# Pablete1234/parquet-floor

Hardware: AMD Instinct MI355X
Metric: decoded GB/s + rows/s (node), lineitem-shape Snappy+dict, 1/2/4/8 GPUs (higher is better)
Workload: dtype u8; 1 GPU; lineitem SF1 x1 (6001215 rows x 1, 16 cols, 6 row groups of 1Mi rows), Snappy + dictionary, device-resident; row_groups_per_rank=6, compressed_page_bytes_rank0=217870360

## Files before the change

parquet-floor_amd/csrc/pf_flat.hip:

```cpp
#include <hip/hip_runtime.h>

#include "pf_flat.h"
#include "pf_flat_chars.h"
#include "pf_launch.h"
#include "pf_snappy_par.h"

namespace pf {

#ifdef PF_STAMPS
#include "pf_stamps.h"
PF_STAMP_TABLE(pf_pstamps, 16, pf_debug_pstamps)
#define PSTAMP(i, v) atomicAdd(&pf_pstamps[i], (unsigned long long)(v))
#else
#define PSTAMP(i, v) ((void)0)
#endif

struct FlatLds {
    uint32_t dpos[DSTR_CAP], dlen[DSTR_CAP];
    Run drun[RUN_CAP];
    Run vrun[RUN_CAP];
    uint32_t coff[FT];
    uint32_t csrc[FT];
    uint16_t cv[CV_CAP];
    uint32_t vbits[FT / 32 + 2];
    uint32_t scan_tmp[NT / 64];
    RunWalk dst, vst;
    int ndrun, nvrun, dres, vres, allp;
    uint32_t dcover, vcover, vlo;
};

#ifndef PF_DICT_LDS
#define PF_DICT_LDS 16384
#endif
constexpr uint32_t DICT_LDS = PF_DICT_LDS;
#ifndef PF_FIX_IDS
#define PF_FIX_IDS 0
#endif
struct FixedLds {
    uint64_t dict[(DICT_LDS + PF_FIX_IDS) / 8 + 2];
    Run vrun[RUN_CAP];
    uint32_t coff[FTX / 64];
    RunWalk vst;
    int nvrun, vres, allp;
    uint32_t vcover, vlo;
    uint32_t ib[2];
};

template <class Lds>
__device__ __forceinline__ int flat_present_fixed(Lds& S, const DevChunk& ck, const DevPage& pg, const Sections& s, bool dict,
                                  bool boolean, int enc, int w, const uint8_t* ids, uint64_t ids_n, int id_bw,
                                  uint64_t slot_base, uint32_t e_begin, uint32_t e_end, bool direct = false) {
    const int tid = threadIdx.x;
    const uint8_t* vend = s.val + s.val_n;
    const bool dalign = dict && (reinterpret_cast<uintptr_t>(ck.dict_data) & uintptr_t(w - 1)) == 0;
    const bool dlds = DICT_LDS > 0 && dict && dalign && (w == 4 || w == 8) && ck.dict_data != nullptr &&
                      ck.dict_n > 0 && uint64_t(ck.dict_n) * uint64_t(w) <= DICT_LDS;
    const uint32_t dbytes = dlds ? (uint32_t(ck.dict_n) * uint32_t(w) + 15u) & ~15u : 0u;
    uint8_t* const sid = reinterpret_cast<uint8_t*>(S.dict) + dbytes;
    int64_t idd = 0;
    bool ilds = false;
    if (dict && dalign && (w == 4 || w == 8) && id_bw > 0 && id_bw <= 32 && s.val_n > 0 && S.vres != 2 &&
        S.vlo <= e_begin && e_end <= S.vcover) {
        if (tid == 0) { S.ib[0] = 0xffffffffu; S.ib[1] = 0u; }
        __syncthreads();
        for (int r = tid; r < S.nvrun; r += NT) {
            const Run R = S.vrun[r];
            const uint32_t f = max(R.first, e_begin), l = min(R.first + R.count, e_end);
            if (!R.packed || f >= l) continue;
            atomicMin(&S.ib[0], uint32_t((uint64_t(R.data) + uint64_t(f - R.first) * uint64_t(id_bw)) >> 3));
            atomicMax(&S.ib[1], uint32_t((uint64_t(R.data) + uint64_t(l - R.first) * uint64_t(id_bw) + 7u) >> 3));
        }
        __syncthreads();
        const uint32_t lo = S.ib[0], hi = S.ib[1];
        if (lo < hi && hi <= ids_n) {
            const uintptr_t a0 = (reinterpret_cast<uintptr_t>(ids) + lo) & ~uintptr_t(15);
            const uintptr_t aend = reinterpret_cast<uintptr_t>(ids) + ids_n;
            const uint32_t nb = (uint32_t(reinterpret_cast<uintptr_t>(ids) + hi - a0) + 8u + 15u) & ~15u;
            if (dbytes + nb <= uint32_t(sizeof(S.dict))) {
                ilds = true;
                idd = int64_t(a0) - int64_t(reinterpret_cast<uintptr_t>(ids));
                for (uint32_t c = tid; c < nb / 16u; c += NT) {
                    const uintptr_t a = a0 + 16u * c;
                    u32x4 x;
                    if (a + 16u <= aend) {
                        x = *reinterpret_cast<const PF_GLOBAL u32x4*>(a);
                    } else {
                        uint32_t q[4] = {0, 0, 0, 0};
                        for (uint32_t b = 0; b < 16u && a + b < aend; b++)
                            q[b >> 2] |= uint32_t(*reinterpret_cast<const PF_GLOBAL uint8_t*>(a + b)) << (8 * (b & 3));
                        x = u32x4{q[0], q[1], q[2], q[3]};
                    }
                    reinterpret_cast<u32x4*>(sid)[c] = x;
                }
            }
        }
    }
    if (dlds) {
        const uint32_t dn = uint32_t(ck.dict_n);
        if (w == 8) {
            const PF_GLOBAL uint64_t* g = (const PF_GLOBAL uint64_t*)(ck.dict_data);
            for (uint32_t i0 = tid; i0 < dn; i0 += 8u * NT) {
                uint64_t v[8];
                #pragma unroll
                for (uint32_t k = 0; k < 8; k++) v[k] = i0 + k * NT < dn ? g[i0 + k * NT] : 0ull;
                #pragma unroll
                for (uint32_t k = 0; k < 8; k++) if (i0 + k * NT < dn) S.dict[i0 + k * NT] = v[k];
            }
        } else {
            const PF_GLOBAL uint32_t* g = (const PF_GLOBAL uint32_t*)(ck.dict_data);
            uint32_t* d32 = reinterpret_cast<uint32_t*>(S.dict);
            for (uint32_t i0 = tid; i0 < dn; i0 += 8u * NT) {
                uint32_t v[8];
                #pragma unroll
                for (uint32_t k = 0; k < 8; k++) v[k] = i0 + k * NT < dn ? g[i0 + k * NT] : 0u;
                #pragma unroll
                for (uint32_t k = 0; k < 8; k++) if (i0 + k * NT < dn) d32[i0 + k * NT] = v[k];
            }
        }
    }
    if (dlds || ilds) __syncthreads();
    for (uint32_t e0 = e_begin, want = 0; e0 < e_end; e0 += want) {
        want = min(uint32_t(FTX), e_end - e0);
        int bad = 0;
        if (dict) {
            if ((S.vlo > e0 || e0 + want > S.vcover) && S.vres == 2) {
                __syncthreads();
                if (tid < 64) {
                    if (tid == 0) { S.vst = RunWalk{0, 0}; S.vlo = e0; }
                    const int rr = wave_walk_runs(ids, ids_n, id_bw, e0, e_end, S.vrun, RUN_CAP, S.nvrun, S.vcover, S.vst, RunWalk{0, 0});
                    if (tid == 0) S.vres = rr;
                }
                __syncthreads();
                if (S.vres == 2 && S.vcover > e0 && e0 + want > S.vcover) want = S.vcover - e0;
            }
            if (id_bw > 32 || s.val_n == 0 || ck.dict_data == nullptr || e0 + want > S.vcover || S.vlo > e0) bad = 1;
            if (!bad && uint32_t(tid) < (want + 63) / 64) S.coff[tid] = uint32_t(run_find(S.vrun, S.nvrun, e0 + tid * 64));
            __syncthreads();
        }
        const bool wide = w == 4 || w == 8;
        if (direct) {
        } else if (!bad && wide && ((dict && dalign) || enc == 0 || enc == 5)) {
#ifndef PF_FB_DIV
#define PF_FB_DIV 2
#endif
            constexpr uint32_t FB = FEPTX / PF_FB_DIV;
            for (uint32_t kb = 0; kb < FEPTX; kb += FB) {
            uint64_t v[FB];
            uint32_t id[FB];
            #pragma unroll
            for (uint32_t k = 0; k < FB; k++) {
                const uint32_t e = e0 + (kb + k) * NT + uint32_t(tid);
                id[k] = 0;
                v[k] = 0;
                if (e >= e0 + want) continue;
                if (dict) {
                    int r = int(S.coff[(e - e0) >> 6]);
                    while (e >= S.vrun[r].first + S.vrun[r].count) r++;
                    const Run R = S.vrun[r];
                    id[k] = R.data;
                    if (R.packed) {
                        const uint64_t bit = uint64_t(R.data) + uint64_t(e - R.first) * uint64_t(id_bw);
                        if (ilds) {
                            const uint32_t rb = uint32_t(int64_t(bit) - 8 * idd);
                            const uint32_t* q = reinterpret_cast<const uint32_t*>(sid) + (rb >> 5);
                            const uint64_t x = (uint64_t(q[0]) | (uint64_t(q[1]) << 32)) >> (rb & 31u);
                            id[k] = uint32_t(x & (id_bw == 32 ? 0xffffffffull : ((1ull << id_bw) - 1ull)));
                        } else {
                            id[k] = (bit >> 3) + 12 <= ids_n ? bits_fast(ids + (bit >> 3), uint32_t(bit & 7), id_bw)
                                                             : bits_le(ids, ids_n, bit, id_bw);
                        }
                    }
                } else if (enc == 0) {
                    if ((uint64_t(e) + 1) * uint64_t(w) > s.val_n) { bad = 1; continue; }
                    const uint8_t* src = s.val + uint64_t(e) * uint64_t(w);
                    if (w == 8) v[k] = src + 12 <= vend ? gld_u64_12(src) : ld64_bytes(src);
                    else v[k] = src + 8 <= vend ? gld_u32_8(src) : ld32le(src, 0, 4);
                } else {
                    v[k] = reinterpret_cast<const uint64_t*>(pg.aux)[e];
                }
            }
            if (dict) {
                const int64_t dn = ck.dict_n;
                #pragma unroll
                for (uint32_t k = 0; k < FB; k++) {
                    const uint32_t e = e0 + (kb + k) * NT + uint32_t(tid);
                    if (e < e0 + want && int64_t(id[k]) >= dn) bad = 1;
                    id[k] = int64_t(id[k]) < dn ? id[k] : 0u;
                }
                if (dlds) {
                    #pragma unroll
                    for (uint32_t k = 0; k < FB; k++)
                        v[k] = w == 8 ? S.dict[id[k]] : reinterpret_cast<const uint32_t*>(S.dict)[id[k]];
                } else if (w == 8) {
                    const PF_GLOBAL uint64_t* g = (const PF_GLOBAL uint64_t*)ck.dict_data;
                    #pragma unroll
                    for (uint32_t k = 0; k < FB; k++) v[k] = g[id[k]];
                } else {
                    const PF_GLOBAL uint32_t* g = (const PF_GLOBAL uint32_t*)ck.dict_data;
                    #pragma unroll
                    for (uint32_t k = 0; k < FB; k++) v[k] = g[id[k]];
                }
            }
            #pragma unroll
            for (uint32_t k = 0; k < FB; k++) {
                const uint32_t e = e0 + (kb + k) * NT + uint32_t(tid);
                if (e >= e0 + want) continue;
                uint8_t* dst = ck.values + (slot_base + e) * uint64_t(w);
                if (w == 8) *reinterpret_cast<uint64_t*>(dst) = v[k];
                else *reinterpret_cast<uint32_t*>(dst) = uint32_t(v[k]);
            }
            }
        } else if (!bad) {
            #pragma unroll 2
            for (uint32_t k = 0; k < FEPTX; k++) {
                const uint32_t e = e0 + k * NT + uint32_t(tid);
                if (e >= e0 + want) break;
                uint8_t* dst = ck.values + (slot_base + e) * uint64_t(w);
                if (dict) {
                    int r = int(S.coff[(e - e0) >> 6]);
                    while (e >= S.vrun[r].first + S.vrun[r].count) r++;
                    const Run R = S.vrun[r];
                    uint32_t id = R.data;
                    if (R.packed) {
                        const uint64_t bit = uint64_t(R.data) + uint64_t(e - R.first) * uint64_t(id_bw);
                        id = (bit >> 3) + 12 <= ids_n ? bits_fast(ids + (bit >> 3), uint32_t(bit & 7), id_bw)
                                                      : bits_le(ids, ids_n, bit, id_bw);
                    }
                    if (int64_t(id) >= ck.dict_n) { bad = 1; continue; }
                    const uint8_t* src = ck.dict_data + uint64_t(id) * uint64_t(w);
                    if (w == 8 && dalign) *reinterpret_cast<uint64_t*>(dst) = *reinterpret_cast<const uint64_t*>(src);
                    else if (w == 4 && dalign) *reinterpret_cast<uint32_t*>(dst) = *reinterpret_cast<const uint32_t*>(src);
                    else copy_value(dst, src, w);
                } else if (boolean) {
                    if ((e >> 3) >= s.val_n) { bad = 1; continue; }
                    dst[0] = uint8_t((s.val[e >> 3] >> (e & 7)) & 1u);
                } else if (enc == 0) {
                    if ((uint64_t(e) + 1) * uint64_t(w) > s.val_n) { bad = 1; continue; }
                    const uint8_t* src = s.val + uint64_t(e) * uint64_t(w);
                    if (w == 8 && src + 12 <= vend) *reinterpret_cast<uint64_t*>(dst) = gld_u64_12(src);
                    else if (w == 4 && src + 8 <= vend) *reinterpret_cast<uint32_t*>(dst) = gld_u32_8(src);
                    else copy_value(dst, src, w);
                } else {
                    const uint64_t* dv = reinterpret_cast<const uint64_t*>(pg.aux);
                    if (w == 8) *reinterpret_cast<uint64_t*>(dst) = dv[e];
                    else *reinterpret_cast<uint32_t*>(dst) = uint32_t(dv[e]);
                }
            }
        }
        if (ck.max_def > 0 && ck.validity) {
            const uint64_t b0 = slot_base + e0, b1 = b0 + want;
            uint32_t* vw = reinterpret_cast<uint32_t*>(ck.validity);
            for (uint64_t wd = (b0 >> 5) + tid; wd <= ((b1 - 1) >> 5); wd += NT) {
                const uint64_t lo = max(b0, wd << 5), hi = min(b1, (wd + 1) << 5);
                const uint32_t m = uint32_t((hi - lo >= 32 ? 0xffffffffull : ((1ull << (hi - lo)) - 1ull)) << (lo & 31));
                if (lo == (wd << 5) && hi == ((wd + 1) << 5)) vw[wd] = m;
                else atomicOr(vw + wd, m);
            }
        }
        if (__syncthreads_or(bad)) return 1;
    }
    return 0;
}

__device__ __forceinline__ bool flat_fixed_block(FixedLds& S, const DevChunk* __restrict__ chunks, DevPage* pages, const int2 pbk,
                                 DevChunkResult* res) {
    if (pbk.x < 0) return true;
    const int pi = pbk.x;
    const uint32_t blk = uint32_t(pbk.y) & 0x0fffffffu;
    const uint32_t bsz = FBLK << (uint32_t(pbk.y) >> 28);
    DevPage& pg = pages[pi];
    const DevChunk& ck = chunks[pg.chunk];
    const int tid = threadIdx.x;
    const int* jfb = pg.jfb;
    const bool dval = pg.direct == DIRECT_VALUES;
    const int jf = jfb != nullptr ? *jfb : FB_WHOLE + 1;
    const int done = pg.done;
    if (done & DONE_DSTR) return true;
    if ((res[pg.chunk].status != 0) | (ck.max_rep != 0) | (ck.ptype == 6) | ((done & DONE_NULL) != 0)) return false;
    if (dval & (jf <= FB_WHOLE)) {
        const uint32_t ne = uint32_t(pg.num_values), e_begin = blk * bsz;
        if (e_begin >= ne && blk > 0) return true;
        const uint32_t e_end = min(ne, e_begin + bsz);
        if (ck.max_def > 0 && ck.validity && e_end > e_begin)
            fill_valid_ones(ck, uint64_t(pg.entry_start) + e_begin, uint64_t(pg.entry_start) + e_end);
        if (threadIdx.x == 0) {
            if (ck.needs_count == 0)
                atomicAdd(reinterpret_cast<unsigned long long*>(&res[pg.chunk].num_values), (unsigned long long)(e_end - e_begin));
            atomicOr(&pg.done, DONE_FIXED);
        }
        return true;
    }
    Sections s;
    if (!page_sections(pg, ck, s)) return false;
    const int enc = pg.encoding;
    const bool boolean = ck.ptype == 0, dict = is_dict_enc(enc);
    const int w = ck.width;
    bool take = ck.max_def == 0 || s.def_rle;
    if (enc == 0) {
    } else if (dict) take = take && !boolean;
    else if (enc == 5) take = take && (ck.ptype == 1 || ck.ptype == 2) && pg.aux != nullptr;
    else take = false;
    if (!take) return false;
    const uint32_t ne = uint32_t(pg.num_values);
    if (blk > 0 && blk * bsz >= ne) return true;
    const int id_bw = (dict && s.val_n > 0) ? int(s.val[0]) : 0;
    const uint8_t* ids = dict && s.val_n > 0 ? s.val + 1 : s.val;
    const uint64_t ids_n = dict && s.val_n > 0 ? s.val_n - 1 : 0;
    const IdRunTab* T = pg.runtab;
    uint32_t t0 = 0, t3 = 0;
    if (T != nullptr) { t0 = T->nruns; t3 = T->all_present; }
    const bool tab = (t3 == 1u) & (t0 <= uint32_t(RUN_CAP));
    if (tid == 0)
        S.allp = tab ? 1 : (ck.max_def == 0 ? 1 : all_present(s.def, s.def_n, bit_width(ck.max_def), ne, uint32_t(ck.max_def)));
    __syncthreads();
    if (!S.allp) return false;
    const uint32_t e_begin = blk * bsz;
    const uint32_t e_end = min(ne, e_begin + bsz);
#ifdef PF_STAMPS
    const unsigned long long ft0 = __builtin_amdgcn_s_memtime();
#endif
    if (dict) {
        if (tab) {
            const uint32_t nr = T->nruns, cov = T->covered;
            for (uint32_t i = tid; i < nr; i += NT) S.vrun[i] = id_run(T, i, nr, cov);
            if (tid == 0) { S.nvrun = int(nr); S.vcover = cov; S.vlo = 0; S.vres = cov >= ne ? 0 : 1; }
        } else if (tid < 64) {
            if (tid == 0) { S.nvrun = 0; S.vcover = 0; S.vres = 0; S.vlo = e_begin; S.vst = RunWalk{0, 0}; }
            if (s.val_n > 0 && id_bw <= 32) {
                const int rr = wave_walk_runs(ids, ids_n, id_bw, e_begin, e_end, S.vrun, RUN_CAP, S.nvrun, S.vcover, S.vst, RunWalk{0, 0});
                if (tid == 0) S.vres = rr;
            }
        }
        __syncthreads();
    }
    const bool direct = dval & (jf <= FB_WHOLE);
    const int err = flat_present_fixed(S, ck, pg, s, dict, boolean, enc, w, ids, ids_n, id_bw,
                                       uint64_t(pg.entry_start), e_begin, e_end, direct);
#ifdef PF_STAMPS
    if (tid == 0) { const unsigned long long dt_ = __builtin_amdgcn_s_memtime() - ft0; PSTAMP(1, dt_); PSTAMP(0, 1); atomicMax(&pf_pstamps[9], dt_); }
#endif
    if (tid == 0) {
        if (err) set_status(res, pg.chunk, ST_CORRUPT, pi);
        else if (ck.needs_count == 0)
            atomicAdd(reinterpret_cast<unsigned long long*>(&res[pg.chunk].num_values), (unsigned long long)(e_end - e_begin));
        atomicOr(&pg.done, DONE_FIXED);
    }
    return true;
}

#ifndef PF_FIXED_OCC
#define PF_FIXED_OCC 6
#endif
__global__ __launch_bounds__(NT, PF_FIXED_OCC) void k_flat_fixed(const DevChunk* __restrict__ chunks, DevPage* pages,
                                                              const int2* __restrict__ blocks, DevChunkResult* res, int* fbq) {
    __shared__ FixedLds S;
    const int2 pbk = blocks[blockIdx.x];
    if (!flat_fixed_block(S, chunks, pages, pbk, res)) null_fallback(fbq, pbk);
}

__device__ __forceinline__ void flat_block(FlatLds& S, const DevChunk* __restrict__ chunks, DevPage* pages, const int2 pbk,
                           DevChunkResult* res) {
    if (pbk.x < 0) return;
    const int pi = pbk.x;
    const uint32_t blk = uint32_t(pbk.y) & 0x0fffffffu;
    const uint32_t bsz = FBLK << (uint32_t(pbk.y) >> 28);
    DevPage& pg = pages[pi];
    const DevChunk& ck = chunks[pg.chunk];
    const int tid = threadIdx.x;
    if ((res[pg.chunk].status != 0) | (ck.max_rep != 0) | ((pg.done & (DONE_FIXED | DONE_NULL | DONE_DSTR)) != 0)) return;
    Sections s;
    if (!page_sections(pg, ck, s)) return;
    const int enc = pg.encoding;
    const bool binary = ck.ptype == 6, boolean = ck.ptype == 0, dict = is_dict_enc(enc);
    const int w = ck.width;
    bool take = ck.max_def == 0 || s.def_rle;
    if (enc == 0) {
    } else if (dict) take = take && !boolean;
    else if (enc == 5) take = take && (ck.ptype == 1 || ck.ptype == 2) && pg.aux != nullptr;
    else take = false;
    if (!take) return;

    const int bwd = bit_width(ck.max_def);
    const uint32_t ne = uint32_t(pg.num_values);
    const int id_bw = (dict && s.val_n > 0) ? int(s.val[0]) : 0;
    const uint8_t* ids = dict && s.val_n > 0 ? s.val + 1 : s.val;
    const uint64_t ids_n = dict && s.val_n > 0 ? s.val_n - 1 : 0;
    const bool counted = ck.needs_count != 0;
    const uint64_t slot_base = uint64_t(pg.entry_start);
    if (blk > 0 && blk * bsz >= ne) return;
    const IdRunTab* T = pg.runtab;
    uint32_t t0 = 0, t3 = 0;
    if (T != nullptr) { t0 = T->nruns; t3 = T->all_present; }
    const bool tab = (t3 == 1u) & (t0 <= uint32_t(RUN_CAP));
    if (tid == 0) S.allp = tab ? 1 : (ck.max_def == 0 ? 1 : all_present(s.def, s.def_n, bwd, ne, uint32_t(ck.max_def)));
    __syncthreads();
    const bool split = S.allp;
    if (!split && blk > 0) return;
    const uint32_t e_begin = split ? blk * bsz : 0u;
    const uint32_t e_end = split ? min(ne, e_begin + bsz) : ne;
#ifdef PF_STAMPS
    const unsigned long long ft0 = __builtin_amdgcn_s_memtime();
    if (tid == 0) { PSTAMP(0, 1); if (dict) PSTAMP(6, 1); if (binary) PSTAMP(7, 1); }
#endif
    if (tid < 64) {
        if (tid == 0) { S.ndrun = 0; S.dcover = ne; S.dres = 0; S.dst = RunWalk{0, 0}; }
        if (!split && ck.max_def > 0) {
            const int rr = wave_walk_runs(s.def, s.def_n, bwd, 0, ne, S.drun, RUN_CAP, S.ndrun, S.dcover, S.dst, RunWalk{0, 0});
            if (tid == 0) S.dres = rr;
        }
    } else if (tid < 128 && !(split && tab)) {
        if (tid == 64) { S.nvrun = 0; S.vcover = 0; S.vres = 0; S.vlo = e_begin; S.vst = RunWalk{0, 0}; }
        if (dict && s.val_n > 0 && id_bw <= 32) {
            const int rr = wave_walk_runs(ids, ids_n, id_bw, e_begin, split ? e_end : ne, S.vrun, RUN_CAP, S.nvrun,
                                          S.vcover, S.vst, RunWalk{0, 0});
            if (tid == 64) S.vres = rr;
        }
    }
    if (split && tab) {
        const uint32_t nr = T->nruns, cov = T->covered;
        for (uint32_t i = tid; i < nr; i += NT) S.vrun[i] = id_run(T, i, nr, cov);
        if (tid == 0) { S.nvrun = int(nr); S.vcover = cov; S.vlo = 0; S.vres = cov >= ne ? 0 : 1; }
    }
    const bool dstage = binary && dict && ck.dict_pos != nullptr && ck.dict_n > 0 && ck.dict_n <= int64_t(DSTR_CAP);
    if (dstage) {
        const PF_GLOBAL uint32_t* gp = gptr(ck.dict_pos);
        const PF_GLOBAL uint32_t* gl = gptr(ck.dict_len);
        for (uint32_t i = uint32_t(tid); i < uint32_t(ck.dict_n); i += NT) { S.dpos[i] = gp[i]; S.dlen[i] = gl[i]; }
    }
    __syncthreads();
#ifdef PF_STAMPS
    unsigned long long ft1 = __builtin_amdgcn_s_memtime();
    if (tid == 0) PSTAMP(2, ft1 - ft0);
#endif
    if (!split && (S.dres == 2 || S.vres == 2)) return;
    bool allp = true, lvl_bad = S.dres != 0;
    if (!split) {
        for (int r = 0; r < S.ndrun; r++) {
            const Run& R = S.drun[r];
            if (R.packed || R.data != uint32_t(ck.max_def)) allp = false;
            if (!R.packed && R.data > uint32_t(ck.max_def)) lvl_bad = true;
        }
    }
    if (lvl_bad) {
        if (tid == 0) { set_status(res, pg.chunk, ST_CORRUPT, pi); atomicOr(&pg.done, DONE_FLAT); }
        return;
    }
    uint64_t char_base = 0;
    if (binary && counted) {
        char_base = uint64_t(pg.char_start);
        if (e_begin > 0) {
            if (dict) char_base += flat_block_chars(pg)[blk];
            else char_base += uint64_t(pg.aux[e_begin]) - 4ull * (uint64_t(e_begin) + 1);
        }
    }
    uint64_t vidx = e_begin;
    int err = 0;
#ifdef PF_STAMPS
    unsigned long long fs_ = __builtin_amdgcn_s_memtime();
#define FSTAMP(i) do { const unsigned long long t_ = __builtin_amdgcn_s_memtime(); if (tid == 0) PSTAMP(i, t_ - fs_); fs_ = t_; } while (0)
#else
#define FSTAMP(i) ((void)0)
#endif


    for (uint32_t e0 = e_begin, want = 0; e0 < e_end; e0 += want) {
        want = min(uint32_t(FT), e_end - e0);
        if (split && dict && S.vres == 2 && (uint64_t(S.vlo) > uint64_t(e0) || e0 + want > S.vcover)) {
            __syncthreads();
            if (tid < 64) {
                if (tid == 0) { S.vst = RunWalk{0, 0}; S.vlo = e0; }
                const int rr = wave_walk_runs(ids, ids_n, id_bw, e0, e_end, S.vrun, RUN_CAP, S.nvrun, S.vcover, S.vst,
                                              RunWalk{0, 0});
                if (tid == 0) S.vres = rr;
            }
            __syncthreads();
            if (S.vres == 2 && S.vcover > e0 && e0 + want > S.vcover) want = S.vcover - e0;
        }
        const uint32_t eb = uint32_t(tid) * FEPT;
        for (uint32_t i = tid; i < FT / 32 + 2; i += NT) S.vbits[i] = 0;
        uint32_t fv = 0;
        int bad = 0;
        if (eb < want) {
            const uint32_t m = min(uint32_t(FEPT), want - eb);
            if (allp) {
                fv = m >= 32 ? 0xffffffffu : (1u << m) - 1u;
            } else {
                const uint32_t e = e0 + eb;
                int r = run_find(S.drun, S.ndrun, e);
                for (uint32_t k = 0; k < m; k++) {
                    while (e + k >= S.drun[r].first + S.drun[r].count) r++;
                    const uint32_t d = run_value(S.drun[r], s.def, s.def_n, e + k, bwd);
                    bad |= d > uint32_t(ck.max_def);
                    fv |= uint32_t(d == uint32_t(ck.max_def)) << k;
                }
            }
        }
        uint32_t tv;
        uint32_t vo;
        if (allp) { vo = min(eb, want); tv = want; }
        else vo = block_excl_scan<NT>(__popc(fv), S.scan_tmp, tv);
        if (tv > 0 && dict) {
            if (split && (uint64_t(S.vlo) > vidx || vidx + tv > uint64_t(S.vcover)) && S.vres == 2) {
                __syncthreads();
                if (tid < 64) {
                    if (tid == 0) { S.vst = RunWalk{0, 0}; S.vlo = uint32_t(vidx); }
                    const int rr = wave_walk_runs(ids, ids_n, id_bw, uint32_t(vidx), e_end, S.vrun, RUN_CAP, S.nvrun,
                                                  S.vcover, S.vst, RunWalk{0, 0});
                    if (tid == 0) S.vres = rr;
                }
                __syncthreads();
            }
            if (id_bw > 32 || s.val_n == 0 || (binary ? ck.dict_pos == nullptr : ck.dict_data == nullptr) ||
                vidx + tv > uint64_t(S.vcover) || uint64_t(S.vlo) > vidx)
                bad = 1;
        }
        if (__syncthreads_or(bad)) { err = 1; break; }
        FSTAMP(11);
        uint32_t lsum = 0;
        uint32_t my_src[FEPT], my_len[FEPT];
        {
            uint32_t j = 0;
            int vr = -1;
            #pragma unroll
            for (uint32_t k = 0; k < FEPT; k++) {
                my_src[k] = 0;
                my_len[k] = 0;
                if (eb + k >= want) continue;
                const uint64_t slot = slot_base + e0 + eb + k;
                const bool present = (fv >> k) & 1u;
                if (!binary) {
                    uint8_t* dst = ck.values + slot * uint64_t(w);
                    if (!present) { zero_value(dst, w); continue; }
                    const uint64_t gv = vidx + vo + j++;
                    if (dict) {
                        if (vr < 0) vr = run_find(S.vrun, S.nvrun, uint32_t(gv));
                        while (gv >= uint64_t(S.vrun[vr].first) + S.vrun[vr].count) vr++;
                        const uint32_t id = run_value(S.vrun[vr], ids, ids_n, uint32_t(gv), id_bw);
                        if (int64_t(id) >= ck.dict_n) { bad = 1; continue; }
                        copy_value(dst, ck.dict_data + uint64_t(id) * uint64_t(w), w);
                    } else if (boolean) {
                        if ((gv >> 3) >= s.val_n) { bad = 1; continue; }
                        dst[0] = uint8_t((s.val[gv >> 3] >> (gv & 7)) & 1u);
                    } else if (enc == 0) {
                        if ((gv + 1) * uint64_t(w) > s.val_n) { bad = 1; continue; }
                        copy_value(dst, s.val + gv * uint64_t(w), w);
                    } else {
                        const uint64_t* dv = reinterpret_cast<const uint64_t*>(pg.aux);
                        if (w == 8) *reinterpret_cast<uint64_t*>(dst) = dv[gv];
                        else *reinterpret_cast<uint32_t*>(dst) = uint32_t(dv[gv]);
                    }
                } else if (present) {
                    const uint64_t gv = vidx + vo + j;
                    if (dict) {
                        if (vr < 0) vr = run_find(S.vrun, S.nvrun, uint32_t(gv));
                        while (gv >= uint64_t(S.vrun[vr].first) + S.vrun[vr].count) vr++;
                        const Run R = S.vrun[vr];
                        uint32_t id = R.data;
                        if (R.packed) {
                            const uint64_t bit = uint64_t(R.data) + uint64_t(uint32_t(gv) - R.first) * uint64_t(id_bw);
                            id = (bit >> 3) + 12 <= ids_n ? bits_fast(ids + (bit >> 3), uint32_t(bit & 7), id_bw)
                                                          : bits_le(ids, ids_n, bit, id_bw);
                        }
                        my_src[k] = id;
                        my_len[k] = 1;
                    } else {
                        const PF_GLOBAL uint32_t* ax = gptr(pg.aux);
                        const uint32_t p = ax[gv];
                        uint32_t ln;
                        if (split && gv + 1 < uint64_t(ne)) {
                            const uint32_t nx = ax[gv + 1];
                            ln = nx >= p + 4 ? nx - p - 4 : 0xffffffffu;
                        } else {
                            ln = (p >= 4 && p <= s.val_n) ? ld32le(s.val, p - 4, s.val_n) : 0xffffffffu;
                        }
                        if (p >= 4 && p <= s.val_n && ln <= s.val_n - p) { my_src[k] = p; my_len[k] = ln; lsum += ln; }
                        else bad = 1;
                    }
                    j++;
                }
            }
            if (binary && dict) {
                const PF_GLOBAL uint32_t* gp = gptr(ck.dict_pos);
                const PF_GLOBAL uint32_t* gl = gptr(ck.dict_len);
                #pragma unroll
                for (uint32_t k = 0; k < FEPT; k++) {
                    if (!my_len[k]) continue;
                    const uint32_t id = my_src[k];
                    uint32_t src = 0, l = 0;
                    if (int64_t(id) >= ck.dict_n) bad = 1;
                    else if (dstage) { src = S.dpos[id]; l = S.dlen[id]; }
                    else { src = gp[id]; l = gl[id]; }
                    my_src[k] = src;
                    my_len[k] = l;
                    lsum += l;
                }
            }
        }
        FSTAMP(12);
        uint32_t tchars = 0;
        const uint32_t lo = binary ? block_excl_scan<NT>(lsum, S.scan_tmp, tchars) : 0;
        if (binary && char_base + tchars > uint64_t(pg.char_start + pg.n_chars)) bad = 1;
        if (__syncthreads_or(bad)) { err = 1; break; }
        FSTAMP(13);
        if (binary) {
            uint32_t c = lo, j = 0;
            #pragma unroll
            for (uint32_t k = 0; k < FEPT; k++) {
                if (eb + k >= want) continue;
                if ((fv >> k) & 1u) {
                    S.coff[vo + j] = c;
                    S.csrc[vo + j] = my_src[k];
                    c += my_len[k];
                    j++;
                }
                ck.offsets[slot_base + e0 + eb + k + 1] = int32_t(char_base + c);
            }
        }
        if (ck.max_def > 0 && fv) {
            const uint64_t abase = (slot_base + e0) & ~uint64_t(31);
            const uint64_t rb = slot_base + e0 + eb - abase;
            const uint32_t sh = uint32_t(rb & 31);
            atomicOr(&S.vbits[rb >> 5], fv << sh);
            if (sh + FEPT > 32 && sh) atomicOr(&S.vbits[(rb >> 5) + 1], fv >> (32 - sh));
        }
        __syncthreads();
#ifdef PF_STAMPS
        { const unsigned long long t_ = __builtin_amdgcn_s_memtime(); if (tid == 0) { PSTAMP(4, t_ - ft1); PSTAMP(3, 1); PSTAMP(14, t_ - fs_); } ft1 = t_; fs_ = t_; }
#endif
        if (binary) {
            const uint8_t* sb = dict ? ck.dict_data : s.val;
            const uint8_t* se = dict ? pages[ck.dict_page].body + pages[ck.dict_page].body_len : s.val + s.val_n;
            if (tchars <= SHORT_AVG * tv) copy_chars_short(S.coff, S.csrc, tv, tchars, sb, ck.chars + char_base);
            else if (!dict) copy_chars_plain(S.coff, S.csrc, tv, tchars, sb, se, ck.chars + char_base, S.cv);
            else copy_chars_fast(S.coff, S.csrc, tv, tchars, sb, se, ck.chars + char_base, S.cv);
        }
        FSTAMP(15);
        if (ck.max_def > 0 && ck.validity) flush_bits(S.vbits, slot_base + e0, want, ck.validity);
        vidx += tv;
        char_base += tchars;
        __syncthreads();
#ifdef PF_STAMPS
        { const unsigned long long t_ = __builtin_amdgcn_s_memtime(); if (tid == 0) PSTAMP(5, t_ - ft1); ft1 = t_; }
#endif
    }
#ifdef PF_STAMPS
    if (tid == 0) {
        const unsigned long long dt_ = __builtin_amdgcn_s_memtime() - ft0;
        PSTAMP(1, dt_);
        atomicMax(&pf_pstamps[binary ? 8 : 9], dt_);
        if (!split) PSTAMP(10, 1);
    }
#endif
    if (tid == 0) {
        if (err) set_status(res, pg.chunk, ST_CORRUPT, pi);
        else if (!counted) atomicAdd(reinterpret_cast<unsigned long long*>(&res[pg.chunk].num_values),
                                     (unsigned long long)(vidx - e_begin));
        atomicOr(&pg.done, DONE_FLAT);
    }
}

#ifndef PF_FLAT_OCC
#define PF_FLAT_OCC 5
#endif
__global__ __launch_bounds__(NT, PF_FLAT_OCC) void k_flat_all(const DevChunk* __restrict__ chunks, DevPage* pages,
                                                 const int2* __restrict__ blocks, int n, const int* __restrict__ fbq,
                                                 DevChunkResult* res) {
    __shared__ union FlatAllLds {
        FixedLds f;
        FlatLds g;
    } S;
    if (int(blockIdx.x) >= n) {
        const int nq = fbq[0], g = int(gridDim.x) - n;
        for (int i = int(blockIdx.x) - n; i < nq; i += g) {
            const int2 pq = reinterpret_cast<const int2*>(fbq + 4)[i];
            if (!flat_fixed_block(S.f, chunks, pages, pq, res)) {
                __syncthreads();
                flat_block(S.g, chunks, pages, pq, res);
            }
            __syncthreads();
        }
        return;
    }
    const int2 pbk = blocks[blockIdx.x];
    if (flat_fixed_block(S.f, chunks, pages, pbk, res)) return;
    __syncthreads();
    flat_block(S.g, chunks, pages, pbk, res);
}

void launch_flat(const DevChunk* d_chunks, DevPage* d_pages, const int* d_list, int nfix, int n, int n4, int n8, int* d_fbq,
                 const int2* d_dblk, int n_dblk, DevChunkResult* d_res, hipStream_t st, NullCaps nc, int stagger) {
    const int2* blocks = reinterpret_cast<const int2*>(d_list);
    launch_flat_null(d_chunks, d_pages, blocks + nfix + n, n4, n8, d_fbq, d_res, st, nc, stagger);
    if (nfix > 0) hipLaunchKernelGGL(k_flat_fixed, dim3(nfix), dim3(NT), 0, st, d_chunks, d_pages, blocks, d_res, d_fbq);
    launch_flat_dstr(d_chunks, d_pages, d_dblk, n_dblk, d_res, st);
    const int nq = nfix + n4 + n8;
    const int nqw = nq < 32 ? nq : 32;
    if (n + nqw > 0)
        hipLaunchKernelGGL(k_flat_all, dim3(n + nqw), dim3(NT), 0, st, d_chunks, d_pages, blocks + nfix, n, d_fbq, d_res);
}

}
```

Baseline: 418.3 decoded GB/s.

## Add 8-values-per-thread dictionary gather fast path for fixed-width flat pages

Adds a specialized path in the fixed-width flat kernel for dictionary-encoded 4/8-byte columns. Each thread decodes 8 consecutive ids, either from a constant RLE run or by unpacking bit-packed words with width-specialized code. It prefetches several groups of packed words ahead, stages the dictionary in LDS when it fits, and writes results with vectorized 16-byte stores. The goal is to cut per-element run lookups and scalar bit extraction. In exchange it costs more registers and code size and keeps a per-element slow path for groups that straddle runs.

```diff
diff --git a/parquet-floor_amd/csrc/pf_fix_ids.h b/parquet-floor_amd/csrc/pf_fix_ids.h
--- /dev/null
+++ b/parquet-floor_amd/csrc/pf_fix_ids.h
@@ -0,0 +1,124 @@
+#pragma once
+#include <stdint.h>
+
+#include "pf_internal.h"
+
+namespace pf {
+
+constexpr int FIX_BW_MAX = 16;
+constexpr int FIX_NDW = 5;
+
+enum : uint32_t { FIX_SLOW = 0, FIX_CONST = 1, FIX_PACKED = 2 };
+struct FixGrp {
+    uint32_t kind;
+    uint32_t val;
+    uint32_t off4;
+};
+
+struct FixRowsRt {
+    const uint32_t* rt;
+    uint32_t nr, cov;
+    PF_HD uint32_t first(uint32_t i) const { return rt[2 * i] & 0x7fffffffu; }
+    PF_HD uint32_t end(uint32_t i) const { return i + 1 < nr ? (rt[2 * i + 2] & 0x7fffffffu) : cov; }
+    PF_HD uint32_t packed(uint32_t i) const { return rt[2 * i] >> 31; }
+    PF_HD uint32_t data(uint32_t i) const { return rt[2 * i + 1]; }
+};
+
+PF_HD inline int fix_ndw(int bw) { return bw > 0 ? (8 * bw + 62) / 32 : 0; }
+
+template <class Rows>
+PF_HD inline FixGrp fix_locate(const Rows& R, uint32_t nr, uint32_t e0, uint32_t n, int bw, uint32_t mis, uint64_t ids_n) {
+    FixGrp g{FIX_SLOW, 0u, 0u};
+    if (nr == 0 || n == 0 || n > 8) return g;
+    uint32_t lo = 0, hi = nr;
+    while (hi - lo > 1) {
+        const uint32_t m = (lo + hi) >> 1;
+        if (R.first(m) <= e0) lo = m; else hi = m;
+    }
+    const uint32_t first = R.first(lo);
+    if (e0 < first || e0 + n > R.end(lo)) return g;
+    if (!R.packed(lo) || bw == 0) {
+        g.kind = FIX_CONST;
+        g.val = R.packed(lo) ? 0u : R.data(lo);
+    } else if (n == 8 && bw <= FIX_BW_MAX) {
+        const uint64_t bit = uint64_t(R.data(lo)) + uint64_t(e0 - first) * uint64_t(bw);
+        const uint64_t o = (bit >> 3) + mis;
+        const uint64_t o4 = o & ~3ull;
+        if (o4 >= mis && o4 + 4u * uint64_t(fix_ndw(bw)) <= uint64_t(mis) + ids_n) {
+            g.kind = FIX_PACKED;
+            g.val = uint32_t(o & 3u) * 8u + uint32_t(bit & 7u);
+            g.off4 = uint32_t(o4);
+        }
+    }
+    return g;
+}
+
+template <class Mem>
+PF_HD inline void fix_load(int bw, uint32_t off4, const Mem& M, uint32_t (&q)[FIX_NDW]) {
+    const int ndw = fix_ndw(bw);
+#ifdef __HIP_DEVICE_COMPILE__
+    #pragma unroll
+#endif
+    for (int i = 0; i < FIX_NDW; i++)
+        if (i < ndw) q[i] = M(off4 + 4u * uint32_t(i));
+}
+
+template <int BW>
+PF_HD inline void fix_unpack_n(const uint32_t (&q)[FIX_NDW], uint32_t pos0, uint32_t (&id)[8]) {
+    static_assert(BW >= 1 && BW <= FIX_BW_MAX, "widths of the fast path");
+    constexpr int NR = (8 * BW + 31) / 32;
+    constexpr uint32_t mask = (1u << BW) - 1u;
+    uint32_t r[NR + 1];
+#ifdef __HIP_DEVICE_COMPILE__
+    #pragma unroll
+#endif
+    for (int i = 0; i < NR; i++) r[i] = uint32_t(((uint64_t(q[i + 1]) << 32) | uint64_t(q[i])) >> pos0);
+    r[NR] = 0;
+#ifdef __HIP_DEVICE_COMPILE__
+    #pragma unroll
+#endif
+    for (int k = 0; k < 8; k++) {
+        const int w = (k * BW) >> 5, s = (k * BW) & 31;
+        uint32_t x = r[w] >> s;
+        if (s + BW > 32) x |= r[w + 1] << ((32 - s) & 31);
+        id[k] = x & mask;
+    }
+}
+PF_HD inline void fix_unpack(int bw, const uint32_t (&q)[FIX_NDW], uint32_t pos0, uint32_t (&id)[8]) {
+    switch (bw) {
+        case 1: fix_unpack_n<1>(q, pos0, id); break;
+        case 2: fix_unpack_n<2>(q, pos0, id); break;
+        case 3: fix_unpack_n<3>(q, pos0, id); break;
+        case 4: fix_unpack_n<4>(q, pos0, id); break;
+        case 5: fix_unpack_n<5>(q, pos0, id); break;
+        case 6: fix_unpack_n<6>(q, pos0, id); break;
+        case 7: fix_unpack_n<7>(q, pos0, id); break;
+        case 8: fix_unpack_n<8>(q, pos0, id); break;
+        case 9: fix_unpack_n<9>(q, pos0, id); break;
+        case 10: fix_unpack_n<10>(q, pos0, id); break;
+        case 11: fix_unpack_n<11>(q, pos0, id); break;
+        case 12: fix_unpack_n<12>(q, pos0, id); break;
+        case 13: fix_unpack_n<13>(q, pos0, id); break;
+        case 14: fix_unpack_n<14>(q, pos0, id); break;
+        case 15: fix_unpack_n<15>(q, pos0, id); break;
+        case 16: fix_unpack_n<16>(q, pos0, id); break;
+        default: break;
+    }
+}
+
+template <class Rows, class Mem>
+PF_HD inline bool fix_ids8(const Rows& R, uint32_t nr, uint32_t e0, uint32_t n, int bw, uint32_t mis, uint64_t ids_n,
+                           const Mem& M, uint32_t (&id)[8]) {
+    const FixGrp g = fix_locate(R, nr, e0, n, bw, mis, ids_n);
+    if (g.kind == FIX_SLOW) return false;
+    if (g.kind == FIX_CONST) {
+        for (int k = 0; k < 8; k++) id[k] = g.val;
+        return true;
+    }
+    uint32_t q[FIX_NDW] = {0, 0, 0, 0, 0};
+    fix_load(bw, g.off4, M, q);
+    fix_unpack(bw, q, g.val, id);
+    return true;
+}
+
+}
diff --git a/parquet-floor_amd/csrc/pf_flat.hip b/parquet-floor_amd/csrc/pf_flat.hip
--- a/parquet-floor_amd/csrc/pf_flat.hip
+++ b/parquet-floor_amd/csrc/pf_flat.hip
@@ -1,5 +1,10 @@
 #include <hip/hip_runtime.h>
 
+#ifdef PF_DIAG
+#include <cstdlib>
+#endif
+
+#include "pf_fix_ids.h"
 #include "pf_flat.h"
 #include "pf_flat_chars.h"
 #include "pf_launch.h"
@@ -262,6 +267,209 @@
     return 0;
 }
 
+#ifdef PF_DIAG
+__device__ unsigned long long pf_fix8_counts[3];
+extern "C" int pf_debug_fix8_counts(unsigned long long* out, int reset) {
+    if (hipMemcpyFromSymbol(out, HIP_SYMBOL(pf_fix8_counts), sizeof(unsigned long long) * 3) != hipSuccess) return -1;
+    if (reset) {
+        const unsigned long long z[3] = {0, 0, 0};
+        if (hipMemcpyToSymbol(HIP_SYMBOL(pf_fix8_counts), z, sizeof z) != hipSuccess) return -1;
+    }
+    return 0;
+}
+#define FIX8_COUNT(i, n) ((void)atomicAdd(&pf_fix8_counts[i], (unsigned long long)(n)))
+#else
+#define FIX8_COUNT(i, n) ((void)0)
+#endif
+
+__device__ __forceinline__ uint32_t fix_bits_pad(const uint8_t* p, uint64_t n, uint64_t bit, int w) {
+    if (w == 0) return 0;
+    const uint64_t by = bit >> 3;
+    const int sh = int(bit & 7);
+    uint64_t acc = 0;
+    #pragma unroll
+    for (int k = 0; k < 5; k++)
+        if (8 * k < sh + w && by + k < n) acc |= uint64_t(p[by + k]) << (8 * k);
+    return uint32_t((acc >> sh) & (w == 32 ? 0xffffffffull : ((1ull << w) - 1)));
+}
+
+constexpr uint32_t FIX_GR = 4;
+
+struct FixRowsLds {
+    const Run* r;
+    __device__ __forceinline__ uint32_t first(uint32_t i) const { return r[i].first; }
+    __device__ __forceinline__ uint32_t end(uint32_t i) const { return r[i].first + r[i].count; }
+    __device__ __forceinline__ uint32_t packed(uint32_t i) const { return r[i].packed; }
+    __device__ __forceinline__ uint32_t data(uint32_t i) const { return r[i].data; }
+};
+struct FixMemGlobal {
+    const PF_GLOBAL uint8_t* base;
+    __device__ __forceinline__ uint32_t operator()(uint32_t o) const { return *reinterpret_cast<const PF_GLOBAL uint32_t*>(base + o); }
+};
+
+template <int LEAD>
+__device__ __forceinline__ void store_vals8(PF_GLOBAL uint32_t* p, const uint32_t (&v)[8]) {
+    #pragma unroll
+    for (int k = 0; k < LEAD; k++) p[k] = v[k];
+    #pragma unroll
+    for (int k = LEAD; k + 4 <= 8; k += 4) *reinterpret_cast<PF_GLOBAL u32x4*>(p + k) = u32x4{v[k], v[k + 1], v[k + 2], v[k + 3]};
+    #pragma unroll
+    for (int k = LEAD + (8 - LEAD) / 4 * 4; k < 8; k++) p[k] = v[k];
+}
+template <int LEAD>
+__device__ __forceinline__ void store_vals8(PF_GLOBAL uint64_t* p, const uint64_t (&v)[8]) {
+    #pragma unroll
+    for (int k = 0; k < LEAD; k++) p[k] = v[k];
+    #pragma unroll
+    for (int k = LEAD; k + 2 <= 8; k += 2)
+        *reinterpret_cast<PF_GLOBAL u32x4*>(p + k) = u32x4{uint32_t(v[k]), uint32_t(v[k] >> 32), uint32_t(v[k + 1]), uint32_t(v[k + 1] >> 32)};
+    #pragma unroll
+    for (int k = LEAD + (8 - LEAD) / 2 * 2; k < 8; k++) p[k] = v[k];
+}
+
+template <class V>
+__device__ __forceinline__ void fixed8_stage_dict(V* sd, const PF_GLOBAL V* gd, uint32_t dn) {
+    for (uint32_t i0 = threadIdx.x; i0 < dn; i0 += 8u * NT) {
+        V v[8];
+        #pragma unroll
+        for (uint32_t k = 0; k < 8; k++) v[k] = i0 + k * NT < dn ? gd[i0 + k * NT] : V(0);
+        #pragma unroll
+        for (uint32_t k = 0; k < 8; k++) if (i0 + k * NT < dn) sd[i0 + k * NT] = v[k];
+    }
+}
+
+template <class V>
+__device__ __forceinline__ void fixed8_gather_store(const V* sd, const PF_GLOBAL V* gd, const uint32_t (&id)[8], PF_GLOBAL V* p,
+                                                    uint32_t n) {
+    V v[8];
+    if (sd != nullptr) {
+        #pragma unroll
+        for (uint32_t k = 0; k < 8; k++) v[k] = sd[id[k]];
+    } else {
+        #pragma unroll
+        for (uint32_t k = 0; k < 8; k++) v[k] = gd[id[k]];
+    }
+    if (n == 8) {
+        constexpr uint32_t per = 16u / sizeof(V);
+        const uint32_t lead = (per - uint32_t((reinterpret_cast<uintptr_t>(p) / sizeof(V)) & (per - 1u))) & (per - 1u);
+        if constexpr (sizeof(V) == 4) {
+            switch (lead) {
+                case 0: store_vals8<0>(p, v); break;
+                case 1: store_vals8<1>(p, v); break;
+                case 2: store_vals8<2>(p, v); break;
+                default: store_vals8<3>(p, v); break;
+            }
+        } else {
+            if (lead == 0) store_vals8<0>(p, v);
+            else store_vals8<1>(p, v);
+        }
+    } else {
+        #pragma unroll
+        for (uint32_t k = 0; k < 8; k++) if (k < n) p[k] = v[k];
+    }
+}
+
+#ifndef PF_FIX8_GLOBAL
+#define PF_FIX8_GLOBAL 0
+#endif
+__device__ __forceinline__ int flat_fixed8(FixedLds& S, const DevChunk& ck, [[maybe_unused]] const IdRunTab* T, int w_,
+                                           const uint8_t* ids, uint64_t ids_n_, int id_bw_, uint64_t slot_base, uint32_t e_begin,
+                                           uint32_t e_end) {
+    const uint32_t tid = threadIdx.x;
+    const int w = __builtin_amdgcn_readfirstlane(w_), id_bw = __builtin_amdgcn_readfirstlane(id_bw_);
+    const uint64_t ids_n = uint32_t(__builtin_amdgcn_readfirstlane(int(uint32_t(ids_n_))));
+    const uint32_t dn = uint32_t(__builtin_amdgcn_readfirstlane(int(uint32_t(ck.dict_n))));
+    const bool dlds = DICT_LDS > 0 && uint64_t(dn) * uint64_t(w) <= DICT_LDS;
+    const uint32_t mis = uint32_t(__builtin_amdgcn_readfirstlane(int(uint32_t(reinterpret_cast<uintptr_t>(ids) & 3u))));
+    const FixMemGlobal frame{(const PF_GLOBAL uint8_t*)(ids) - mis};
+    const uint32_t nr = uint32_t(S.nvrun);
+#if PF_FIX8_GLOBAL
+    const FixRowsRt rows{T->rows, nr, S.vcover};
+#else
+    const FixRowsLds rows{S.vrun};
+#endif
+    int bad = 0;
+    [[maybe_unused]] uint32_t nslow = 0;
+    for (uint32_t eb = e_begin; eb < e_end; eb += FIX_GR * 8u * NT) {
+        uint32_t q[FIX_GR][FIX_NDW];
+        uint32_t meta[FIX_GR];
+        #pragma unroll
+        for (uint32_t g = 0; g < FIX_GR; g++) {
+            #pragma unroll
+            for (int i = 0; i < FIX_NDW; i++) q[g][i] = 0;
+            meta[g] = FIX_SLOW << 8;
+            const uint32_t e0 = eb + 8u * (tid + NT * g);
+            if (e0 < e_end) {
+                const FixGrp G = fix_locate(rows, nr, e0, min(8u, e_end - e0), id_bw, mis, ids_n);
+                if (G.kind == FIX_CONST) q[g][0] = G.val;
+                else if (G.kind == FIX_PACKED) fix_load(id_bw, G.off4, frame, q[g]);
+                meta[g] = (G.kind << 8) | (G.kind == FIX_PACKED ? G.val : 0u);
+            }
+        }
+        if (eb == e_begin && dlds) {
+            if (w == 8) fixed8_stage_dict(S.dict, (const PF_GLOBAL uint64_t*)(ck.dict_data), dn);
+            else fixed8_stage_dict(reinterpret_cast<uint32_t*>(S.dict), (const PF_GLOBAL uint32_t*)(ck.dict_data), dn);
+            __syncthreads();
+        }
+        #pragma unroll 1
+        for (uint32_t g = 0; g < FIX_GR; g++) {
+            const uint32_t e0 = eb + 8u * (tid + NT * g);
+            if (e0 < e_end) {
+                const uint32_t n = min(8u, e_end - e0), kind = meta[0] >> 8;
+                uint32_t id[8];
+                if (kind == FIX_PACKED) {
+                    fix_unpack(id_bw, q[0], meta[0] & 0xffu, id);
+                } else if (kind == FIX_CONST) {
+                    #pragma unroll
+                    for (uint32_t k = 0; k < 8; k++) id[k] = q[0][0];
+                } else {
+                    nslow++;
+                    int r = run_find(S.vrun, S.nvrun, e0);
+                    #pragma unroll
+                    for (uint32_t k = 0; k < 8; k++) {
+                        id[k] = 0;
+                        if (k >= n) continue;
+                        const uint32_t e = e0 + k;
+                        while (e >= S.vrun[r].first + S.vrun[r].count) r++;
+                        const Run R = S.vrun[r];
+                        id[k] = R.data;
+                        if (R.packed) {
+                            const uint64_t bit = uint64_t(R.data) + uint64_t(e - R.first) * uint64_t(id_bw);
+                            id[k] = (bit >> 3) + 12 <= ids_n ? bits_fast(ids + (bit >> 3), uint32_t(bit & 7), id_bw)
+                                                             : fix_bits_pad(ids, ids_n, bit, id_bw);
+                        }
+                    }
+                }
+                #pragma unroll
+                for (uint32_t k = 0; k < 8; k++) {
+                    if (k < n && id[k] >= dn) bad = 1;
+                    id[k] = id[k] < dn ? id[k] : 0u;
+                }
+                if (w == 8)
+                    fixed8_gather_store<uint64_t>(dlds ? S.dict : nullptr, (const PF_GLOBAL uint64_t*)(ck.dict_data), id,
+                                                  (PF_GLOBAL uint64_t*)(ck.values) + slot_base + e0, n);
+                else
+                    fixed8_gather_store<uint32_t>(dlds ? reinterpret_cast<const uint32_t*>(S.dict) : nullptr,
+                                                  (const PF_GLOBAL uint32_t*)(ck.dict_data), id,
+                                                  (PF_GLOBAL uint32_t*)(ck.values) + slot_base + e0, n);
+            }
+            #pragma unroll
+            for (uint32_t h = 0; h + 1 < FIX_GR; h++) {
+                meta[h] = meta[h + 1];
+                #pragma unroll
+                for (int i = 0; i < FIX_NDW; i++) q[h][i] = q[h + 1][i];
+            }
+        }
+    }
+    if (ck.max_def > 0 && ck.validity) fill_valid_ones(ck, slot_base + e_begin, slot_base + e_end);
+#ifdef PF_DIAG
+    if (nslow) FIX8_COUNT(1, nslow);
+    if (tid == 0) FIX8_COUNT(0, 1);
+#endif
+    return __syncthreads_or(bad) ? 1 : 0;
+}
+
+template <int MODE>
 __device__ __forceinline__ bool flat_fixed_block(FixedLds& S, const DevChunk* __restrict__ chunks, DevPage* pages, const int2 pbk,
                                  DevChunkResult* res) {
     if (pbk.x < 0) return true;
@@ -334,8 +542,23 @@
         __syncthreads();
     }
     const bool direct = dval & (jf <= FB_WHOLE);
-    const int err = flat_present_fixed(S, ck, pg, s, dict, boolean, enc, w, ids, ids_n, id_bw,
-                                       uint64_t(pg.entry_start), e_begin, e_end, direct);
+    int err;
+    if constexpr (MODE == 1) {
+        const bool fix8 = dict && tab && !direct && (w == 4 || w == 8) && ck.dict_data != nullptr && ck.dict_n > 0 &&
+                          (reinterpret_cast<uintptr_t>(ck.dict_data) & uintptr_t(w - 1)) == 0 && S.vres == 0 &&
+                          id_bw <= FIX_BW_MAX && s.val_n > 0;
+        if (fix8) {
+            err = flat_fixed8(S, ck, T, w, ids, ids_n, id_bw, uint64_t(pg.entry_start), e_begin, e_end);
+        } else {
+            if (dict && tid == 0) FIX8_COUNT(2, 1);
+            err = flat_present_fixed(S, ck, pg, s, dict, boolean, enc, w, ids, ids_n, id_bw,
+                                     uint64_t(pg.entry_start), e_begin, e_end, direct);
+        }
+    } else {
+        if constexpr (MODE == 2) { if (dict && tid == 0) FIX8_COUNT(2, 1); }
+        err = flat_present_fixed(S, ck, pg, s, dict, boolean, enc, w, ids, ids_n, id_bw,
+                                 uint64_t(pg.entry_start), e_begin, e_end, direct);
+    }
 #ifdef PF_STAMPS
     if (tid == 0) { const unsigned long long dt_ = __builtin_amdgcn_s_memtime() - ft0; PSTAMP(1, dt_); PSTAMP(0, 1); atomicMax(&pf_pstamps[9], dt_); }
 #endif
@@ -355,8 +578,16 @@
                                                               const int2* __restrict__ blocks, DevChunkResult* res, int* fbq) {
     __shared__ FixedLds S;
     const int2 pbk = blocks[blockIdx.x];
-    if (!flat_fixed_block(S, chunks, pages, pbk, res)) null_fallback(fbq, pbk);
-}
+    if (!flat_fixed_block<1>(S, chunks, pages, pbk, res)) null_fallback(fbq, pbk);
+}
+#ifdef PF_DIAG
+__global__ __launch_bounds__(NT, PF_FIXED_OCC) void k_flat_fixed_old(const DevChunk* __restrict__ chunks, DevPage* pages,
+                                                                  const int2* __restrict__ blocks, DevChunkResult* res, int* fbq) {
+    __shared__ FixedLds S;
+    const int2 pbk = blocks[blockIdx.x];
+    if (!flat_fixed_block<2>(S, chunks, pages, pbk, res)) null_fallback(fbq, pbk);
+}
+#endif
 
 __device__ __forceinline__ void flat_block(FlatLds& S, const DevChunk* __restrict__ chunks, DevPage* pages, const int2 pbk,
                            DevChunkResult* res) {
@@ -673,7 +904,7 @@
         const int nq = fbq[0], g = int(gridDim.x) - n;
         for (int i = int(blockIdx.x) - n; i < nq; i += g) {
             const int2 pq = reinterpret_cast<const int2*>(fbq + 4)[i];
-            if (!flat_fixed_block(S.f, chunks, pages, pq, res)) {
+            if (!flat_fixed_block<0>(S.f, chunks, pages, pq, res)) {
                 __syncthreads();
                 flat_block(S.g, chunks, pages, pq, res);
             }
@@ -682,7 +913,7 @@
         return;
     }
     const int2 pbk = blocks[blockIdx.x];
-    if (flat_fixed_block(S.f, chunks, pages, pbk, res)) return;
+    if (flat_fixed_block<0>(S.f, chunks, pages, pbk, res)) return;
     __syncthreads();
     flat_block(S.g, chunks, pages, pbk, res);
 }
@@ -691,6 +922,12 @@
                  const int2* d_dblk, int n_dblk, DevChunkResult* d_res, hipStream_t st, NullCaps nc, int stagger) {
     const int2* blocks = reinterpret_cast<const int2*>(d_list);
     launch_flat_null(d_chunks, d_pages, blocks + nfix + n, n4, n8, d_fbq, d_res, st, nc, stagger);
+#ifdef PF_DIAG
+    const char* fix8_env = std::getenv("PF_FIX8");
+    if (nfix > 0 && fix8_env && fix8_env[0] == '0')
+        hipLaunchKernelGGL(k_flat_fixed_old, dim3(nfix), dim3(NT), 0, st, d_chunks, d_pages, blocks, d_res, d_fbq);
+    else
+#endif
     if (nfix > 0) hipLaunchKernelGGL(k_flat_fixed, dim3(nfix), dim3(NT), 0, st, d_chunks, d_pages, blocks, d_res, d_fbq);
     launch_flat_dstr(d_chunks, d_pages, d_dblk, n_dblk, d_res, st);
     const int nq = nfix + n4 + n8;
```

After: 426.1 decoded GB/s (median of 6 runs). +1.9%, better.
